# KarelPeeters/kZero

Hardware: AMD Instinct MI355X
Metric: self-play NN evals/sec (node), Chess 20x256 ResNet b=256, 1/2/4/8 GPU (higher is better)
Workload: dtype f16; 1 GPU; chess-20x256 attention head, executor batch 256; engines_per_gpu=1, parallelism=dp1 (no collective)

## Files before the change

kzero_amd/csrc/kz_encode_dev.hpp:

```cpp
#pragma once

__device__ __forceinline__ float encoded_plane(const PackedBoards in, int board, int ch, int square, int hw) {
    float f = 0.0f;
    if (ch < in.n_scalar) {
        f = in.scalars[(size_t)board * in.n_scalar + ch];
    } else if (ch < in.n_scalar + in.n_bool) {
        const uint8_t *bb = in.bits + (size_t)board * in.stride;
        if (in.sym) square = in.square_src[min((int)in.sym[board], in.n_sym - 1) * hw + square];
        const unsigned bit = (unsigned)(ch - in.n_scalar) * hw + square;
        f = (float)((bb[bit >> 3] >> (bit & 7)) & 1);
    }
    return f;
}
```

kzero_amd/csrc/kz_tower.hip:

```cpp
#include <cstdlib>
#include <type_traits>
#include <vector>

#include "kz_kernels.hpp"
#include "kz_launch.hpp"

namespace kz {

typedef _Float16 h16;
typedef h16 h16x8 __attribute__((ext_vector_type(8)));
typedef h16 h16x4 __attribute__((ext_vector_type(4)));
typedef float f32x4 __attribute__((ext_vector_type(4)));

namespace {

#include "kz_decode_dev.hpp"
#include "kz_encode_dev.hpp"

constexpr int C = 256;
constexpr int RS = C * 2 + 16;
constexpr int URS = 3 * C * 2 + 16;
constexpr int KSTEPS = 72;
constexpr int HEAD_KSTEPS = 5 * 8;
constexpr int POLICY = 1880, LOGIT_LD = 96;
constexpr int TOWER_PF_MAX = 8;

struct TowerDev {
    const h16 *x0;
    const uint4 *w_stem, *w_tower;
    const float *bias, *post_scale, *post_shift;
    h16 *y;
    int cin_p, batch, depth;
    PackedBoards in;
    const float *sh_w0, *sh_b0, *sh_w1, *sh_b1, *sh_w2, *sh_b2;
    const int32_t *att_idx;
    float *scalars, *policy;
    int *nonfinite_flag;
    int epoch;
    DecodeDev dec;
};

template <int I, int N, class F>
__device__ __forceinline__ void static_for(F &&f) {
    if constexpr (I < N) {
        f(std::integral_constant<int, I>{});
        static_for<I + 1, N>(f);
    }
}

template <int NB>
struct Layout {
    static constexpr int M = NB * 64;
    static constexpr int MT = M / 16;
    static constexpr bool LINE_TILES = NB == 2;
    static constexpr int BPAD = LINE_TILES ? 128 : 0;
    static constexpr int BOARD = 64 * RS + BPAD;
    static constexpr int TS = LINE_TILES ? 8 * RS : 16 * RS;
    static constexpr int IMG = NB * BOARD;
    static constexpr int X_OFF = 0;
    static constexpr int Y_OFF = IMG;
    static constexpr int Z_OFF = 2 * IMG;
    static_assert(Z_OFF % 256 == 0, "zero rows keep the slot pattern of the image rows");
    static constexpr int S_OFF = Z_OFF + 16 * RS;
    static constexpr int TOWER_BYTES = S_OFF + M * 64;
    static constexpr int U_OFF = Z_OFF;
    static constexpr int ACT_OFF = U_OFF + 16 * URS;
    static constexpr int HID_OFF = ACT_OFF + NB * 256 * 4;
    static constexpr int HEADS_BYTES = HID_OFF + NB * 32 * 4;
    static constexpr int LOG_OFF = Y_OFF;
    static constexpr int BYTES = TOWER_BYTES > HEADS_BYTES ? TOWER_BYTES : HEADS_BYTES;
    static_assert(NB * 64 * LOGIT_LD * 4 <= IMG, "logits fit the Y region");
    static constexpr int row_off(int b, int p) { return b * BOARD + p * RS; }
    static_assert(BYTES <= 160 * 1024, "LDS budget");
};

constexpr int SG_VALU = 0x2, SG_SALU = 0x4, SG_MFMA = 0x8, SG_VMEM_READ = 0x20, SG_DS_READ = 0x100;

template <int NB, bool HEADS, int PF, bool WIDE = false, bool PREV = false>
__global__ __launch_bounds__(256, 1) void kz_tower_resident(TowerDev a) {
    using L = Layout<NB>;
    constexpr int M = L::M, MT = L::MT;
    static_assert(PF <= TOWER_PF_MAX, "the refills past the end of the stream must land in its padding");
    extern __shared__ __attribute__((aligned(16))) unsigned char lds[];

    const int tid = threadIdx.x;
    const int wave = __builtin_amdgcn_readfirstlane(tid >> 6);
    const int lane = tid & 63;
    const int fr = lane & 15, kq = lane >> 4;
    const int board0 = blockIdx.x * NB;
    const int layers = 2 * a.depth;
    const int total_ksteps = layers * KSTEPS + (HEADS ? HEAD_KSTEPS : 0);
    const int bias_rows = layers + (HEADS ? 5 : 0);

    const uint4 *wp = a.w_tower + wave * 256 + lane;
    auto wload_prev = [&](int gk, int nt) __attribute__((always_inline)) { return wp[(size_t)gk * 1024 + nt * 64]; };
    typedef const __attribute__((address_space(1))) unsigned char *gptr;
    gptr wk = (gptr)a.w_tower + wave * 4096;
    const unsigned wlane = lane * 16;
    auto wload = [&](gptr k, int nt) __attribute__((always_inline)) {
        typedef unsigned u32x4 __attribute__((ext_vector_type(4)));
        return __builtin_bit_cast(uint4, *reinterpret_cast<const __attribute__((address_space(1))) u32x4 *>(k + wlane + nt * 1024));
    };
    uint4 wreg[PF][4];
#pragma unroll
    for (int s = 0; s < PF; s++) {
        const int g = s < total_ksteps ? s : total_ksteps - 1;
#pragma unroll
        for (int nt = 0; nt < 4; nt++) wreg[s][nt] = PREV ? wload_prev(g, nt) : wload(wk + s * 16384, nt);
    }
    wk += PF * 16384;
    int g = 0;
    auto ring_take = [&](int stage, h16x8 (&af)[4]) __attribute__((always_inline)) {
#pragma unroll
        for (int nt = 0; nt < 4; nt++) af[nt] = *reinterpret_cast<const h16x8 *>(&wreg[stage][nt]);
#ifndef KZ_TW_NO_WLOAD
        if constexpr (PREV) {
            const int gn = g + PF < total_ksteps ? g + PF : total_ksteps - 1;
#pragma unroll
            for (int nt = 0; nt < 4; nt++) wreg[stage][nt] = wload_prev(gn, nt);
        } else {
#pragma unroll
            for (int nt = 0; nt < 4; nt++) wreg[stage][nt] = wload(wk, nt);
        }
#endif
        wk += 16384;
        if constexpr (!PREV) asm("" : "+s"(wk));
    };

    const int sc = WIDE ? a.cin_p >> 5 : 1;
    const int stem_off = WIDE ? L::Y_OFF : L::S_OFF, srow = 64 * sc, spieces = 4 * sc;
    for (int id = tid; id < 16 * RS / 16; id += 256)
        *reinterpret_cast<uint4 *>(lds + L::Z_OFF + id * 16) = make_uint4(0, 0, 0, 0);
    for (int id = tid; id < M * spieces; id += 256) {
        const int row = WIDE ? id / spieces : id >> 2, c = id - row * spieces;
        const int board = board0 + (row >> 6);
        uint4 v = make_uint4(0, 0, 0, 0);
        if (board < a.batch) {
            if (a.in.bits) {
                h16x8 e;
#pragma unroll
                for (int j = 0; j < 8; j++) e[j] = (h16)encoded_plane(a.in, board, c * 8 + j, row & 63, 64);
                v = *reinterpret_cast<const uint4 *>(&e);
            } else {
                v = *reinterpret_cast<const uint4 *>(a.x0 + ((size_t)board0 * 64 + row) * a.cin_p + c * 8);
            }
        }
        *reinterpret_cast<uint4 *>(lds + stem_off + row * srow + c * 16) = v;
    }
    __syncthreads();

    f32x4 acc[4][MT];
    f32x4 bias_next[4];
    auto fetch_bias = [&](int row) __attribute__((always_inline)) {
        const int l = row <= bias_rows ? row : bias_rows;
#pragma unroll
        for (int nt = 0; nt < 4; nt++)
            bias_next[nt] = *reinterpret_cast<const f32x4 *>(a.bias + l * C + wave * 64 + nt * 16 + kq * 4);
    };
    auto init_acc = [&]() __attribute__((always_inline)) {
#pragma unroll
        for (int nt = 0; nt < 4; nt++)
#pragma unroll
            for (int mt = 0; mt < MT; mt++) acc[nt][mt] = bias_next[nt];
    };
    f32x4 post_s[4], post_t[4];
#pragma unroll
    for (int nt = 0; nt < 4; nt++) {
        post_s[nt] = f32x4{1.f, 1.f, 1.f, 1.f};
        post_t[nt] = f32x4{0.f, 0.f, 0.f, 0.f};
    }

    auto relu4 = [](f32x4 v) {
        typedef int i32x4 __attribute__((ext_vector_type(4)));
        i32x4 b = __builtin_bit_cast(i32x4, v);
#pragma unroll
        for (int j = 0; j < 4; j++) b[j] = b[j] > 0 ? b[j] : 0;
        return __builtin_bit_cast(f32x4, b);
    };
    auto to_h4 = [](f32x4 v) { return h16x4{(h16)v[0], (h16)v[1], (h16)v[2], (h16)v[3]}; };

    const int lane_row = L::LINE_TILES ? (fr >> 3) * L::BOARD + (fr & 7) * RS : fr * RS;
    const int epi_base = lane_row + (wave * 64 + kq * 4) * 2;
    auto epilogue = [&](int dst_off, auto relu, auto residual, auto post) __attribute__((always_inline)) {
#pragma unroll
        for (int nt = 0; nt < 4; nt++) {
            h16x4 rx[MT];
            if constexpr (decltype(residual)::value) {
#pragma unroll
                for (int mt = 0; mt < MT; mt++)
                    rx[mt] = *reinterpret_cast<const h16x4 *>(lds + L::X_OFF + epi_base + mt * L::TS + nt * 32);
            }
#pragma unroll
            for (int mt = 0; mt < MT; mt++) {
                const int off = epi_base + mt * L::TS + nt * 32;
                f32x4 v = acc[nt][mt];
                if constexpr (decltype(relu)::value) v = relu4(v);
                if constexpr (decltype(residual)::value) {
#pragma unroll
                    for (int j = 0; j < 4; j++) v[j] += (float)rx[mt][j];
                }
                if constexpr (decltype(post)::value) v = v * post_s[nt] + post_t[nt];
                *reinterpret_cast<h16x4 *>(lds + dst_off + off) = to_h4(v);
            }
        }
    };
    constexpr std::true_type YES{};
    constexpr std::false_type NO{};

    const bool x_is0 = (lane & 7) == 0, x_is7 = (lane & 7) == 7, yo_is0 = (lane & 8) == 0, yo_is1 = !yo_is0;
    auto tap_ok = [&](int mt, int dy, int dx) __attribute__((always_inline)) {
        const bool kill_x = (dx < 0 && x_is0) || (dx > 0 && x_is7);
        if constexpr (L::LINE_TILES) return !(kill_x || (dy < 0 && mt == 0) || (dy > 0 && mt == MT - 1));
        else return !(kill_x || ((mt & 3) == 0 && dy < 0 && yo_is0) || ((mt & 3) == 3 && dy > 0 && yo_is1));
    };

    fetch_bias(0);
    init_acc();
    fetch_bias(1);
    for (int ks = 0; ks < 9 * sc; ks++) {
        const int tap = WIDE ? ks / sc : ks, chunk = ks - tap * sc;
        const int dy = tap / 3 - 1, dx = tap % 3 - 1;
        h16x8 af[4];
#pragma unroll
        for (int nt = 0; nt < 4; nt++) {
            const uint4 t = a.w_stem[((ks * 4 + wave) * 4 + nt) * 64 + lane];
            af[nt] = *reinterpret_cast<const h16x8 *>(&t);
        }
#pragma unroll
        for (int mt = 0; mt < MT; mt++) {
            const bool ok = tap_ok(mt, dy, dx);
            const int p = L::LINE_TILES ? (fr >> 3) * 64 + mt * 8 + (fr & 7) : mt * 16 + fr;
            const int off = ok ? stem_off + (p + dy * 8 + dx) * srow + chunk * 64 + kq * 16 : L::Z_OFF + kq * 16;
            const h16x8 bf = *reinterpret_cast<const h16x8 *>(lds + off);
#pragma unroll
            for (int nt = 0; nt < 4; nt++)
                acc[nt][mt] = __builtin_amdgcn_mfma_f32_16x16x32_f16(af[nt], bf, acc[nt][mt], 0, 0, 0);
        }
    }
    epilogue(L::X_OFF, NO, NO, NO);
    __syncthreads();

    const int kq_off = 256 * (kq & 1) + 128 * (kq >> 1);
    const int frag_base = lane_row + kq_off;
    auto tap_rows = [&](int dy, int dx, int src_off, int (&T)[MT]) __attribute__((always_inline)) {
        const int shifted = frag_base + src_off + (dy * 8 + dx) * RS;
        const int zrow = L::Z_OFF + ((fr + dy * 8 + dx) & 15) * RS + kq_off;
        const int zrow_odd = L::LINE_TILES ? L::Z_OFF + ((fr + dy * 8 + dx + 8) & 15) * RS + kq_off : zrow;
        if constexpr (PREV) {
#pragma unroll
            for (int mt = 0; mt < MT; mt++) T[mt] = tap_ok(mt, dy, dx) ? shifted + mt * L::TS : ((mt & 1) ? zrow_odd : zrow);
        } else {
            int z0 = zrow, z1 = zrow_odd;
            asm("" : "+v"(z0), "+v"(z1));
            const bool kill_x = ((dx < 0) & x_is0) | ((dx > 0) & x_is7);
#pragma unroll
            for (int mt = 0; mt < MT; mt++) {
                bool kill = kill_x;
                if constexpr (!L::LINE_TILES) kill = kill_x | (((mt & 3) == 0) & (dy < 0) & yo_is0) | (((mt & 3) == 3) & (dy > 0) & yo_is1);
                T[mt] = kill ? ((mt & 1) ? z1 : z0) : shifted + mt * L::TS;
            }
        }
    };

    h16x8 bf[2][MT];
    constexpr auto tile_lo = [](int dy) { return L::LINE_TILES && dy < 0 ? 1 : 0; };
    constexpr auto tile_hi = [](int dy) { return L::LINE_TILES && dy > 0 ? MT - 1 : MT; };

    auto conv_plain = [&](auto ndy_tag, int src_off, int dx_lo, int dx_hi) __attribute__((always_inline)) {
        constexpr int NDY = decltype(ndy_tag)::value, DY0 = NDY == 3 ? -1 : 0;
        int T[NDY][MT], Tn[NDY][MT];
#pragma unroll
        for (int i = 0; i < NDY; i++) tap_rows(DY0 + i, dx_lo, src_off, T[i]);
#pragma unroll
        for (int mt = tile_lo(DY0); mt < tile_hi(DY0); mt++) bf[0][mt] = *reinterpret_cast<const h16x8 *>(lds + T[0][mt]);
#pragma nounroll
        for (int dx = dx_lo; dx < dx_hi; dx++) {
#pragma unroll
            for (int i = 0; i < NDY; i++) tap_rows(DY0 + i, dx + 1 < dx_hi ? dx + 1 : dx, src_off, Tn[i]);
            static_for<0, 8 * NDY>([&](auto s_tag) __attribute__((always_inline)) {
                constexpr int s = decltype(s_tag)::value, ch = s / NDY, i = s % NDY, dy = DY0 + i;
                constexpr int stage = s & (PF - 1), cur = s & 1, nxt = cur ^ 1;
                constexpr int lo = tile_lo(dy), hi = tile_hi(dy), nt_ = hi - lo;
                constexpr int in_ = (i + 1) % NDY, chn = i + 1 < NDY ? ch : ch + 1;
                constexpr int lon = tile_lo(DY0 + in_), hin = tile_hi(DY0 + in_), nr = hin - lon;
#ifndef KZ_TW_NO_DSREAD
#pragma unroll
                for (int mt = 0; mt < MT; mt++) {
                    if (mt >= lon && mt < hin)
                        bf[nxt][mt] = *reinterpret_cast<const h16x8 *>(lds + (chn < 8 ? T[in_][mt] + chn * 16 : Tn[in_][mt]));
                }
#endif
                h16x8 af[4];
                ring_take(stage, af);
#pragma unroll
                for (int nt = 0; nt < 4; nt++)
#pragma unroll
                    for (int mt = 0; mt < MT; mt++)
                        if (mt >= lo && mt < hi)
                            acc[nt][mt] = __builtin_amdgcn_mfma_f32_16x16x32_f16(af[nt], bf[cur][mt], acc[nt][mt], 0, 0, 0);
#pragma unroll
                for (int j = 0; j < 4; j++) {
                    __builtin_amdgcn_sched_group_barrier(SG_MFMA, 1, 0);
                    __builtin_amdgcn_sched_group_barrier(SG_VMEM_READ, 1, 0);
                }
#pragma unroll
                for (int j = 0; j < MT; j++) {
                    if (j < nr) {
                        __builtin_amdgcn_sched_group_barrier(SG_MFMA, 1, 0);
                        __builtin_amdgcn_sched_group_barrier(SG_DS_READ, 1, 0);
                    }
                }
                constexpr int n_free = 4 * nt_ - (nr + 4), n_alu = PREV || s != 0 ? 0 : n_free < 20 ? n_free : 20;
#pragma unroll
                for (int j = 0; j < 20; j++) {
                    if (j < n_alu) {
                        __builtin_amdgcn_sched_group_barrier(SG_MFMA, 1, 0);
                        __builtin_amdgcn_sched_group_barrier(SG_VALU | SG_SALU, 2, 0);
                    }
                }
                __builtin_amdgcn_sched_group_barrier(SG_MFMA, n_free - n_alu, 0);
                __builtin_amdgcn_sched_barrier(0);
                g++;
            });
#pragma unroll
            for (int i = 0; i < NDY; i++)
#pragma unroll
                for (int mt = 0; mt < MT; mt++) T[i][mt] = Tn[i][mt];
        }
    };

    auto conv_3x3_lines = [&](int src_off) __attribute__((always_inline)) {
        static_assert(!L::LINE_TILES || MT == 8, "one tile per board line");
        int T[MT], Tn[MT];
        tap_rows(0, -1, src_off, T);
#pragma unroll
        for (int mt = 0; mt < MT; mt++) bf[0][mt] = *reinterpret_cast<const h16x8 *>(lds + T[mt]);
#pragma nounroll
        for (int dx = -1; dx < 2; dx++) {
            tap_rows(0, dx < 1 ? dx + 1 : dx, src_off, Tn);
            static_for<0, 8>([&](auto ch_tag) __attribute__((always_inline)) {
                constexpr int ch = decltype(ch_tag)::value, cur = ch & 1, nxt = cur ^ 1;
#ifndef KZ_TW_NO_DSREAD
#pragma unroll
                for (int mt = 0; mt < MT; mt++)
                    bf[nxt][mt] = *reinterpret_cast<const h16x8 *>(lds + (ch < 7 ? T[mt] + (ch + 1) * 16 : Tn[mt]));
#endif
                static_for<0, 3>([&](auto i_tag) __attribute__((always_inline)) {
                    constexpr int i = decltype(i_tag)::value, dy = i - 1, stage = (ch * 3 + i) & (PF - 1);
                    constexpr int lo = tile_lo(dy), hi = tile_hi(dy), nt_ = hi - lo;
                    h16x8 af[4];
                    ring_take(stage, af);
#pragma unroll
                    for (int nt = 0; nt < 4; nt++)
#pragma unroll
                        for (int mt = 0; mt < MT; mt++)
                            if (mt >= lo && mt < hi)
                                acc[nt][mt] = __builtin_amdgcn_mfma_f32_16x16x32_f16(af[nt], bf[cur][mt + dy], acc[nt][mt], 0, 0, 0);
#pragma unroll
                    for (int j = 0; j < 4; j++) {
                        __builtin_amdgcn_sched_group_barrier(SG_MFMA, 1, 0);
                        __builtin_amdgcn_sched_group_barrier(SG_VMEM_READ, 1, 0);
                    }
                    constexpr int nr = i == 0 ? MT : 0;
#pragma unroll
                    for (int j = 0; j < MT; j++) {
                        if (j < nr) {
                            __builtin_amdgcn_sched_group_barrier(SG_MFMA, 1, 0);
                            __builtin_amdgcn_sched_group_barrier(SG_DS_READ, 1, 0);
                        }
                    }
                    constexpr int n_free = 4 * nt_ - (nr + 4), n_alu = ch == 0 && i == 0 ? n_free : 0;
#pragma unroll
                    for (int j = 0; j < 4 * MT; j++) {
                        if (j < n_alu) {
                            __builtin_amdgcn_sched_group_barrier(SG_MFMA, 1, 0);
                            __builtin_amdgcn_sched_group_barrier(SG_VALU | SG_SALU, 2, 0);
                        }
                    }
                    __builtin_amdgcn_sched_group_barrier(SG_MFMA, n_free - n_alu, 0);
                    __builtin_amdgcn_sched_barrier(0);
                    g++;
                });
            });
#pragma unroll
            for (int mt = 0; mt < MT; mt++) T[mt] = Tn[mt];
        }
    };
    constexpr std::integral_constant<int, 3> THREE_ROWS{};
    constexpr std::integral_constant<int, 1> ONE_ROW{};
    auto conv_3x3 = [&](int src_off) __attribute__((always_inline)) {
        if constexpr (L::LINE_TILES && !PREV) conv_3x3_lines(src_off);
        else conv_plain(THREE_ROWS, src_off, -1, 2);
    };
    auto conv_1x1 = [&](int src_off) __attribute__((always_inline)) { conv_plain(ONE_ROW, src_off, 0, 1); };

    for (int layer = 1; layer <= layers; layer++) {
        const bool is_b = (layer & 1) == 0;
        init_acc();
        fetch_bias(layer + 1);
        if (layer == layers) {
#pragma unroll
            for (int nt = 0; nt < 4; nt++) {
                const int oc = wave * 64 + nt * 16 + kq * 4;
                post_s[nt] = *reinterpret_cast<const f32x4 *>(a.post_scale + oc);
                post_t[nt] = *reinterpret_cast<const f32x4 *>(a.post_shift + oc);
            }
        }
        conv_3x3(is_b ? L::Y_OFF : L::X_OFF);
        if (!is_b) epilogue(L::Y_OFF, YES, NO, NO);
        else if (layer != layers) epilogue(L::X_OFF, YES, YES, NO);
        else epilogue(L::X_OFF, YES, YES, YES);
        __syncthreads();
    }

    if constexpr (!HEADS) {
        for (int id = tid; id < M * 32; id += 256) {
            const int p = id >> 5, c16 = id & 31;
            const int board = board0 + (p >> 6);
            if (board < a.batch) {
                const uint4 v = *reinterpret_cast<const uint4 *>(lds + L::X_OFF + L::row_off(p >> 6, p & 63) + c16 * 16);
                *reinterpret_cast<uint4 *>(a.y + ((size_t)board0 * 64 + p) * C + c16 * 8) = v;
            }
        }
    } else {
        {
            float *act = reinterpret_cast<float *>(lds + L::ACT_OFF);
            for (int o = tid; o < NB * 256; o += 256) {
                const int b = o >> 8, c4 = (o >> 6) & 3, p = o & 63;
                const unsigned char *row = lds + L::X_OFF + L::row_off(b, p);
                const float *w = a.sh_w0 + c4 * C;
                float s = a.sh_b0[c4];
#pragma unroll 4
                for (int i = 0; i < C; i += 8) {
                    const h16x8 xv = *reinterpret_cast<const h16x8 *>(row + i * 2);
                    const f32x4 w0 = *reinterpret_cast<const f32x4 *>(w + i), w1 = *reinterpret_cast<const f32x4 *>(w + i + 4);
#pragma unroll
                    for (int j = 0; j < 4; j++) s += (float)xv[j] * w0[j] + (float)xv[4 + j] * w1[j];
                }
                if (!(fabsf(s) <= 3.0e38f) && a.nonfinite_flag && board0 + b < a.batch) {
                    *reinterpret_cast<volatile int *>(a.nonfinite_flag) = a.epoch;
                    raise_nonfinite_board(a.nonfinite_flag, a.epoch, board0 + b);
                }
                act[o] = fmaxf(s, 0.0f);
            }
        }

        {
            const int tb = L::X_OFF + L::row_off(NB == 2 ? fr >> 3 : 0, 56 + (fr & 7)) + kq_off;
            for (int s = 0; s < 3; s++) {
                f32x4 ua[4];
#pragma unroll
                for (int nt = 0; nt < 4; nt++) ua[nt] = bias_next[nt];
                fetch_bias(layers + 2 + s);
#pragma unroll
                for (int ch = 0; ch < 8; ch++) {
                    const h16x8 bf = *reinterpret_cast<const h16x8 *>(lds + tb + ch * 16);
                    h16x8 af[4];
                    ring_take(ch & (PF - 1), af);
#pragma unroll
                    for (int nt = 0; nt < 4; nt++)
                        ua[nt] = __builtin_amdgcn_mfma_f32_16x16x32_f16(af[nt], bf, ua[nt], 0, 0, 0);
                    g++;
                }
                if (NB == 2 || fr < 8) {
#pragma unroll
                    for (int nt = 0; nt < 4; nt++)
                        *reinterpret_cast<h16x4 *>(lds + L::U_OFF + fr * URS + (256 * s + wave * 64 + nt * 16 + kq * 4) * 2) =
                            to_h4(ua[nt]);
                }
            }
        }

        init_acc();
        fetch_bias(layers + 5);
        conv_1x1(L::X_OFF);
        epilogue(L::Y_OFF, NO, NO, NO);

        init_acc();
        conv_1x1(L::X_OFF);
        __syncthreads();
        epilogue(L::X_OFF, NO, NO, NO);
        __syncthreads();

        {
            const float *act = reinterpret_cast<const float *>(lds + L::ACT_OFF);
            float *hid = reinterpret_cast<float *>(lds + L::HID_OFF);
            if (tid < NB * 128) {
                const int pair = tid >> 2, part = tid & 3, b = pair >> 5, j = pair & 31;
                const float *w = a.sh_w1 + j * 256 + part * 64;
                const float *x = act + b * 256 + part * 64;
                float s = 0.0f;
#pragma unroll 4
                for (int i = 0; i < 64; i += 4) {
                    const f32x4 wv = *reinterpret_cast<const f32x4 *>(w + i), xv = *reinterpret_cast<const f32x4 *>(x + i);
                    s += wv[0] * xv[0] + wv[1] * xv[1] + wv[2] * xv[2] + wv[3] * xv[3];
                }
                s += __shfl_xor(s, 1, 64);
                s += __shfl_xor(s, 2, 64);
                if (part == 0) hid[b * 32 + j] = fmaxf(s + a.sh_b1[j], 0.0f);
            }
        }

        constexpr int IT = NB == 2 ? 2 : 1;
        const int hb = NB == 2 ? wave >> 1 : 0;
        const int it0 = NB == 2 ? (wave & 1) * 2 : wave;
        f32x4 la[IT][6];
        {
            int ja[6], ia[IT];
#pragma unroll
            for (int jt = 0; jt < 4; jt++) ja[jt] = L::X_OFF + L::row_off(hb, jt * 16 + fr) + kq_off;
            ja[4] = L::U_OFF + (hb * 8 + (fr & 7)) * URS + (fr >> 3) * 512 + kq_off;
            ja[5] = L::U_OFF + (hb * 8 + (fr & 7)) * URS + 2 * 512 + kq_off;
#pragma unroll
            for (int ii = 0; ii < IT; ii++) ia[ii] = L::Y_OFF + L::row_off(hb, (it0 + ii) * 16 + fr) + kq_off;
#pragma unroll
            for (int ii = 0; ii < IT; ii++)
#pragma unroll
                for (int jt = 0; jt < 6; jt++) la[ii][jt] = f32x4{0.f, 0.f, 0.f, 0.f};
#pragma unroll
            for (int ch = 0; ch < 8; ch++) {
                h16x8 qa[6], qb[IT];
#pragma unroll
                for (int jt = 0; jt < 6; jt++) qa[jt] = *reinterpret_cast<const h16x8 *>(lds + ja[jt] + ch * 16);
#pragma unroll
                for (int ii = 0; ii < IT; ii++) qb[ii] = *reinterpret_cast<const h16x8 *>(lds + ia[ii] + ch * 16);
#pragma unroll
                for (int ii = 0; ii < IT; ii++)
#pragma unroll
                    for (int jt = 0; jt < 6; jt++)
                        la[ii][jt] = __builtin_amdgcn_mfma_f32_16x16x32_f16(qa[jt], qb[ii], la[ii][jt], 0, 0, 0);
            }
        }
        __syncthreads();
        {
            const float inv = 1.0f / sqrtf((float)C);
#pragma unroll
            for (int ii = 0; ii < IT; ii++)
#pragma unroll
                for (int jt = 0; jt < 6; jt++) {
                    const int i = (it0 + ii) * 16 + fr, j = jt * 16 + kq * 4;
                    *reinterpret_cast<f32x4 *>(lds + L::LOG_OFF + ((hb * 64 + i) * LOGIT_LD + j) * 4) = la[ii][jt] * inv;
                }
        }
        const bool decode = a.dec.move_offsets != nullptr;
        float *raw = reinterpret_cast<float *>(lds + L::ACT_OFF);
        if (tid < NB * 5) {
            const int b = tid / 5, k = tid % 5;
            const float *hid = reinterpret_cast<const float *>(lds + L::HID_OFF) + b * 32;
            float s = a.sh_b2[k];
            for (int i = 0; i < 32; i++) s += a.sh_w2[k * 32 + i] * hid[i];
            if (decode) raw[b * 8 + k] = s;
            else if (board0 + b < a.batch) a.scalars[(size_t)(board0 + b) * 5 + k] = s;
        }
        __syncthreads();
        if (decode) {
            if (wave < NB && board0 + wave < a.batch) {
                const float *lg = reinterpret_cast<const float *>(lds + L::LOG_OFF) + wave * 64 * LOGIT_LD;
                float *stage = reinterpret_cast<float *>(lds + L::X_OFF + L::row_off(wave, 0));
                decode_board_wave(a.dec, board0 + wave, lane, raw + wave * 8, stage, 64 * RS / 4,
                                  [&](int idx) { return lg[a.att_idx[idx]]; });
            }
        } else {
            for (int b = 0; b < NB; b++) {
                if (board0 + b >= a.batch) break;
                const float *lg = reinterpret_cast<const float *>(lds + L::LOG_OFF) + b * 64 * LOGIT_LD;
                float *pol = a.policy + (size_t)(board0 + b) * POLICY;
                for (int k = tid; k < POLICY; k += 256) pol[k] = lg[a.att_idx[k]];
            }
        }
    }
}

#ifndef KZ_PF_NB1
#define KZ_PF_NB1 4
#endif
#ifndef KZ_PF_NB2
#define KZ_PF_NB2 4
#endif
constexpr int PF_NB1 = KZ_PF_NB1, PF_NB2 = KZ_PF_NB2;

void pack_1x1(const float *w, uint16_t *dst) {
    static const int kq_base[4] = {0, 128, 64, 192};
    for (int chunk = 0; chunk < 8; chunk++)
        for (int wave = 0; wave < 4; wave++)
            for (int nt = 0; nt < 4; nt++)
                for (int lane = 0; lane < 64; lane++)
                    for (int j = 0; j < 8; j++) {
                        const int oc = 64 * wave + 16 * nt + (lane & 15);
                        const int ch = 8 * chunk + kq_base[lane >> 4] + j;
                        const _Float16 hv = (_Float16)w[(size_t)oc * 256 + ch];
                        uint16_t bits;
                        __builtin_memcpy(&bits, &hv, 2);
                        dst[((((size_t)chunk * 4 + wave) * 4 + nt) * 64 + lane) * 8 + j] = bits;
                    }
}

}

bool tower_resident_supported(int dtype, int h, int w, int channels, int depth, int c_in) {
    return dtype == 1 && h == 8 && w == 8 && channels == C && depth >= 1 && c_in >= 1 && c_in <= 224;
}

bool tower_heads_supported(int policy_kind, int query_channels, int policy_len, int sh_channels, int sh_size) {
    return policy_kind == 2 && query_channels == C && policy_len == POLICY && sh_channels == 4 && sh_size == 32;
}

size_t tower_packed_weight_elems(int cin_p, int depth) {
    return (size_t)9 * C * cin_p + (size_t)2 * depth * 9 * C * C;
}

size_t tower_heads_weight_elems() { return (size_t)HEAD_KSTEPS * 16 * 1024 / 2; }

size_t tower_weight_pad_elems() { return (size_t)TOWER_PF_MAX * 16 * 1024 / 2; }

void tower_pack_weights(const float *oihw, int cout, int cin, int cin_p, uint16_t *dst, bool tap_major) {
    const int nchunk = cin_p / 32;
    const bool rows_inner = cin_p == 256 && !tap_major;
    static const int kq_base[4] = {0, 128, 64, 192};
    for (int tap = 0; tap < 9; tap++)
        for (int chunk = 0; chunk < nchunk; chunk++) {
            const size_t kstep = rows_inner ? ((size_t)(tap % 3) * 8 + chunk) * 3 + tap / 3 : (size_t)tap * nchunk + chunk;
            for (int wave = 0; wave < 4; wave++)
                for (int nt = 0; nt < 4; nt++)
                    for (int lane = 0; lane < 64; lane++)
                        for (int j = 0; j < 8; j++) {
                            const int oc = 64 * wave + 16 * nt + (lane & 15);
                            const int kq = lane >> 4;
                            const int ch = cin_p == 256 ? 8 * chunk + kq_base[kq] + j : 32 * chunk + 8 * kq + j;
                            float v = 0.0f;
                            if (oc < cout && ch < cin) v = oihw[((size_t)oc * cin + ch) * 9 + tap];
                            const _Float16 hv = (_Float16)v;
                            uint16_t bits;
                            __builtin_memcpy(&bits, &hv, 2);
                            dst[(((kstep * 4 + wave) * 4 + nt) * 64 + lane) * 8 + j] = bits;
                        }
        }
}

void tower_pack_heads(const float *w_bulk , const float *b_bulk, const float *w_under ,
                      const float *b_under, uint16_t *dst, float *bias5) {
    const size_t pass = (size_t)8 * 16 * 1024 / 2;
    std::vector<float> tmp((size_t)256 * 256);
    for (int s = 0; s < 3; s++) {
        for (int q = 0; q < 256; q++) {
            for (int c = 0; c < 256; c++) tmp[(size_t)q * 256 + c] = w_under[(size_t)(3 * q + s) * 256 + c];
            bias5[s * 256 + q] = b_under[3 * q + s];
        }
        pack_1x1(tmp.data(), dst + pass * s);
    }
    pack_1x1(w_bulk, dst + pass * 3);
    pack_1x1(w_bulk + (size_t)256 * 256, dst + pass * 4);
    for (int q = 0; q < 256; q++) {
        bias5[3 * 256 + q] = b_bulk[q];
        bias5[4 * 256 + q] = b_bulk[256 + q];
    }
}

namespace {
template <auto Kernel>
void launch_instance(const TowerDev &d, int grid, int bytes, hipStream_t stream) {
    allow_dynamic_lds<Kernel>(bytes);
    Kernel<<<grid, 256, bytes, stream>>>(d);
}
}

void launch_tower_resident(const TowerArgs &t, hipStream_t stream) {
    TowerDev d{};
    d.x0 = static_cast<const h16 *>(t.x0);
    d.w_stem = static_cast<const uint4 *>(t.w_stem);
    d.w_tower = static_cast<const uint4 *>(t.w_tower);
    d.bias = t.bias;
    d.post_scale = t.post_scale;
    d.post_shift = t.post_shift;
    d.y = static_cast<h16 *>(t.y);
    d.cin_p = t.cin_p;
    d.batch = t.batch;
    d.depth = t.depth;
    d.in = t.in;
    d.sh_w0 = t.sh_w0; d.sh_b0 = t.sh_b0; d.sh_w1 = t.sh_w1; d.sh_b1 = t.sh_b1; d.sh_w2 = t.sh_w2; d.sh_b2 = t.sh_b2;
    d.att_idx = t.att_idx;
    d.scalars = t.scalars;
    d.policy = t.policy;
    d.nonfinite_flag = t.nonfinite_flag;
    d.epoch = t.epoch;
    d.dec = decode_dev(t.decode, t.fused_heads, POLICY);
    const bool heads = t.fused_heads;
#ifdef KZ_EXPERIMENTS
    if (t.prev) {
        const int grid = (t.batch + 1) / 2;
        if (t.cin_p > 32) {
            if (heads) launch_instance<kz_tower_resident<2, true, PF_NB2, true, true>>(d, grid, Layout<2>::BYTES, stream);
            else launch_instance<kz_tower_resident<2, false, PF_NB2, true, true>>(d, grid, Layout<2>::BYTES, stream);
        } else if (t.boards_per_wg == 1) {
            if (heads) launch_instance<kz_tower_resident<1, true, PF_NB1, false, true>>(d, t.batch, Layout<1>::BYTES, stream);
            else launch_instance<kz_tower_resident<1, false, PF_NB1, false, true>>(d, t.batch, Layout<1>::BYTES, stream);
        } else {
            if (heads) launch_instance<kz_tower_resident<2, true, PF_NB2, false, true>>(d, grid, Layout<2>::BYTES, stream);
            else launch_instance<kz_tower_resident<2, false, PF_NB2, false, true>>(d, grid, Layout<2>::BYTES, stream);
        }
        return;
    }
#endif
    if (t.cin_p > 32) {
        const int grid = (t.batch + 1) / 2;
        if (heads) launch_instance<kz_tower_resident<2, true, PF_NB2, true>>(d, grid, Layout<2>::BYTES, stream);
        else launch_instance<kz_tower_resident<2, false, PF_NB2, true>>(d, grid, Layout<2>::BYTES, stream);
    } else if (t.boards_per_wg == 1) {
        if (heads) launch_instance<kz_tower_resident<1, true, PF_NB1>>(d, t.batch, Layout<1>::BYTES, stream);
        else launch_instance<kz_tower_resident<1, false, PF_NB1>>(d, t.batch, Layout<1>::BYTES, stream);
    } else {
        const int grid = (t.batch + 1) / 2;
        if (heads) launch_instance<kz_tower_resident<2, true, PF_NB2>>(d, grid, Layout<2>::BYTES, stream);
        else launch_instance<kz_tower_resident<2, false, PF_NB2>>(d, grid, Layout<2>::BYTES, stream);
    }
}

}
```

Before: 551,600 evals/s.

## Stage packed board bits in LDS before encoding; use scalar loads for head weights

The resident tower kernel now loads each block's packed bitboards, scalars and symmetry ids into registers before the weight prefetch, then writes them into the X image region of LDS. The stem encode reads bits from LDS instead of issuing scattered global byte loads per plane. Separately, the shared-head first layer indexes weights by wave through the constant address space, which lets the compiler use scalar loads since c4 is wave-uniform. This adds a sync and some register pressure, and depends on the LDS scratch fitting the X image, which a static_assert checks.

Result: no change. 553,100 evals/s, median of 6 (+0.3%).

```diff
diff --git a/kzero_amd/csrc/kz_encode_dev.hpp b/kzero_amd/csrc/kz_encode_dev.hpp
--- a/kzero_amd/csrc/kz_encode_dev.hpp
+++ b/kzero_amd/csrc/kz_encode_dev.hpp
@@ -12,3 +12,128 @@
     }
     return f;
 }
+
+struct EncodeScratch {
+    int bits_bytes, slot, scal_off, sym_off;
+};
+
+__device__ __forceinline__ EncodeScratch encode_scratch(const PackedBoards in, int hw, int nb) {
+    EncodeScratch s;
+    s.bits_bytes = (in.n_bool * hw + 7) >> 3;
+    s.slot = (s.bits_bytes + 3) & ~3;
+    s.scal_off = nb * s.slot;
+    s.sym_off = s.scal_off + nb * in.n_scalar * 4;
+    return s;
+}
+constexpr int encode_scratch_max_bytes(int planes, int hw, int nb) {
+    return nb * (((planes * hw + 7) / 8 + 3) / 4 * 4 + planes * 4 + 1);
+}
+
+template <int NB, int U>
+struct EncodeStaged {
+    uint32_t w[U];
+    float s[2];
+    uint32_t id;
+    int nb;
+    bool dwords;
+};
+
+template <int NB>
+__device__ __forceinline__ int encode_stage_row(int i, int wpr) {
+    int row = 0;
+#pragma unroll
+    for (int k = 1; k < NB; k++) row += i >= k * wpr;
+    return row;
+}
+
+template <int NB, int U>
+__device__ __forceinline__ void encode_stage_issue(const PackedBoards in, int board0, int batch, int hw, int tid,
+                                                   int nthreads, EncodeStaged<NB, U> &r) {
+    const EncodeScratch L = encode_scratch(in, hw, NB);
+    r.nb = min(NB, batch - board0);
+    r.dwords = (((uintptr_t)in.bits | (uintptr_t)in.stride | (uintptr_t)L.bits_bytes) & 3) == 0;
+    const uint8_t *base = in.bits + (size_t)board0 * in.stride;
+    const int wpr = r.dwords ? L.bits_bytes >> 2 : L.bits_bytes, total = r.nb * wpr;
+    if (total > 0) {
+        if (r.dwords) {
+#pragma unroll
+            for (int u = 0; u < U; u++) {
+                const int i = min(tid + u * nthreads, total - 1), row = encode_stage_row<NB>(i, wpr);
+                r.w[u] = *reinterpret_cast<const uint32_t *>(base + (size_t)row * in.stride + (size_t)(i - row * wpr) * 4);
+            }
+        } else {
+#pragma unroll
+            for (int u = 0; u < U; u++) {
+                const int i = min(tid + u * nthreads, total - 1), row = encode_stage_row<NB>(i, wpr);
+                r.w[u] = base[(size_t)row * in.stride + (i - row * wpr)];
+            }
+        }
+    }
+    const int total_s = r.nb * in.n_scalar;
+    if (total_s > 0) {
+        const float *sc = in.scalars + (size_t)board0 * in.n_scalar;
+#pragma unroll
+        for (int u = 0; u < 2; u++) r.s[u] = sc[min(tid + u * nthreads, total_s - 1)];
+    }
+    if (in.sym) r.id = in.sym[board0 + min(tid, r.nb - 1)];
+}
+
+template <int NB, int U>
+__device__ __forceinline__ void encode_stage_commit(const PackedBoards in, int board0, int hw, int tid, int nthreads,
+                                                    const EncodeStaged<NB, U> &r, unsigned char *scratch) {
+    const EncodeScratch L = encode_scratch(in, hw, NB);
+    const uint8_t *base = in.bits + (size_t)board0 * in.stride;
+    const int wpr = r.dwords ? L.bits_bytes >> 2 : L.bits_bytes, total = r.nb * wpr;
+    if (r.dwords) {
+#pragma unroll
+        for (int u = 0; u < U; u++) {
+            const int i = tid + u * nthreads, row = encode_stage_row<NB>(i, wpr);
+            if (i < total) *reinterpret_cast<uint32_t *>(scratch + row * L.slot + (i - row * wpr) * 4) = r.w[u];
+        }
+#pragma nounroll
+        for (int i = tid + U * nthreads; i < total; i += nthreads) {
+            const int row = encode_stage_row<NB>(i, wpr), col = i - row * wpr;
+            *reinterpret_cast<uint32_t *>(scratch + row * L.slot + col * 4) =
+                *reinterpret_cast<const uint32_t *>(base + (size_t)row * in.stride + (size_t)col * 4);
+        }
+    } else {
+#pragma unroll
+        for (int u = 0; u < U; u++) {
+            const int i = tid + u * nthreads, row = encode_stage_row<NB>(i, wpr);
+            if (i < total) scratch[row * L.slot + (i - row * wpr)] = (uint8_t)r.w[u];
+        }
+#pragma nounroll
+        for (int i = tid + U * nthreads; i < total; i += nthreads) {
+            const int row = encode_stage_row<NB>(i, wpr), col = i - row * wpr;
+            scratch[row * L.slot + col] = base[(size_t)row * in.stride + col];
+        }
+    }
+    const int total_s = r.nb * in.n_scalar;
+    float *ss = reinterpret_cast<float *>(scratch + L.scal_off);
+    const float *sc = in.scalars + (size_t)board0 * in.n_scalar;
+#pragma unroll
+    for (int u = 0; u < 2; u++) {
+        const int i = tid + u * nthreads;
+        if (i < total_s) ss[i] = r.s[u];
+    }
+#pragma nounroll
+    for (int i = tid + 2 * nthreads; i < total_s; i += nthreads) ss[i] = sc[i];
+    if (in.sym && tid < r.nb) scratch[L.sym_off + tid] = (uint8_t)r.id;
+}
+
+__device__ __forceinline__ int encoded_square_staged(const PackedBoards in, const EncodeScratch L, const unsigned char *scratch,
+                                                     int b, int square, int hw) {
+    if (in.sym) square = in.square_src[min((int)scratch[L.sym_off + b], in.n_sym - 1) * hw + square];
+    return square;
+}
+
+__device__ __forceinline__ float encoded_plane_staged(const PackedBoards in, const EncodeScratch L, const unsigned char *scratch,
+                                                      int b, int ch, int sq, int hw) {
+    const int cs = max(min(ch, in.n_scalar - 1), 0), pl = max(min(ch - in.n_scalar, in.n_bool - 1), 0);
+    const float fs = reinterpret_cast<const float *>(scratch + L.scal_off)[b * in.n_scalar + cs];
+    const unsigned bit = (unsigned)pl * hw + sq;
+    unsigned byte = scratch[b * L.slot + (bit >> 3)];
+    asm volatile("" : "+v"(byte));
+    const float fb = (float)((byte >> (bit & 7)) & 1);
+    return ch < in.n_scalar ? fs : ch < in.n_scalar + in.n_bool ? fb : 0.0f;
+}
diff --git a/kzero_amd/csrc/kz_tower.hip b/kzero_amd/csrc/kz_tower.hip
--- a/kzero_amd/csrc/kz_tower.hip
+++ b/kzero_amd/csrc/kz_tower.hip
@@ -92,6 +92,11 @@
     const int total_ksteps = layers * KSTEPS + (HEADS ? HEAD_KSTEPS : 0);
     const int bias_rows = layers + (HEADS ? 5 : 0);
 
+    constexpr int STAGE_U = 4;
+    static_assert(encode_scratch_max_bytes(224, 64, NB) <= L::IMG, "the raw boards fit the X image");
+    EncodeStaged<NB, STAGE_U> staged{};
+    if (a.in.bits) encode_stage_issue(a.in, board0, a.batch, 64, tid, 256, staged);
+
     const uint4 *wp = a.w_tower + wave * 256 + lane;
     auto wload_prev = [&](int gk, int nt) __attribute__((always_inline)) { return wp[(size_t)gk * 1024 + nt * 64]; };
     typedef const __attribute__((address_space(1))) unsigned char *gptr;
@@ -131,6 +136,12 @@
     const int stem_off = WIDE ? L::Y_OFF : L::S_OFF, srow = 64 * sc, spieces = 4 * sc;
     for (int id = tid; id < 16 * RS / 16; id += 256)
         *reinterpret_cast<uint4 *>(lds + L::Z_OFF + id * 16) = make_uint4(0, 0, 0, 0);
+    const unsigned char *raw_boards = lds + L::X_OFF;
+    const EncodeScratch es = encode_scratch(a.in, 64, NB);
+    if (a.in.bits) {
+        encode_stage_commit(a.in, board0, 64, tid, 256, staged, lds + L::X_OFF);
+        __syncthreads();
+    }
     for (int id = tid; id < M * spieces; id += 256) {
         const int row = WIDE ? id / spieces : id >> 2, c = id - row * spieces;
         const int board = board0 + (row >> 6);
@@ -138,8 +149,9 @@
         if (board < a.batch) {
             if (a.in.bits) {
                 h16x8 e;
-#pragma unroll
-                for (int j = 0; j < 8; j++) e[j] = (h16)encoded_plane(a.in, board, c * 8 + j, row & 63, 64);
+                const int sq = encoded_square_staged(a.in, es, raw_boards, row >> 6, row & 63, 64);
+#pragma unroll
+                for (int j = 0; j < 8; j++) e[j] = (h16)encoded_plane_staged(a.in, es, raw_boards, row >> 6, c * 8 + j, sq, 64);
                 v = *reinterpret_cast<const uint4 *>(&e);
             } else {
                 v = *reinterpret_cast<const uint4 *>(a.x0 + ((size_t)board0 * 64 + row) * a.cin_p + c * 8);
@@ -425,15 +437,18 @@
     } else {
         {
             float *act = reinterpret_cast<float *>(lds + L::ACT_OFF);
+            typedef const __attribute__((address_space(4))) float *cfptr;
+            typedef const __attribute__((address_space(4))) f32x4 *cf4ptr;
+            const cfptr w = (cfptr)a.sh_w0 + wave * C;
+            const float b0 = ((cfptr)a.sh_b0)[wave];
             for (int o = tid; o < NB * 256; o += 256) {
-                const int b = o >> 8, c4 = (o >> 6) & 3, p = o & 63;
+                const int b = o >> 8, p = o & 63;
                 const unsigned char *row = lds + L::X_OFF + L::row_off(b, p);
-                const float *w = a.sh_w0 + c4 * C;
-                float s = a.sh_b0[c4];
+                float s = b0;
 #pragma unroll 4
                 for (int i = 0; i < C; i += 8) {
                     const h16x8 xv = *reinterpret_cast<const h16x8 *>(row + i * 2);
-                    const f32x4 w0 = *reinterpret_cast<const f32x4 *>(w + i), w1 = *reinterpret_cast<const f32x4 *>(w + i + 4);
+                    const f32x4 w0 = *reinterpret_cast<cf4ptr>(w + i), w1 = *reinterpret_cast<cf4ptr>(w + i + 4);
 #pragma unroll
                     for (int j = 0; j < 4; j++) s += (float)xv[j] * w0[j] + (float)xv[4 + j] * w1[j];
                 }
```
